# mbway/turbo

Hardware: AMD Instinct MI355X
Metric: acquisition evals/sec (M candidates, N training) + GP-fit ms (higher is better)
Workload: dtype f32

## Files before the change

turbo_amd/_lib.py:

```python
import ctypes
import importlib.util
import os
import sys

import numpy as np

_HERE = os.path.dirname(os.path.abspath(__file__))

os.environ.setdefault("GPU_MAX_HW_QUEUES", "8")
LIB_PATH = os.environ.get("TGP_LIBRARY") or os.path.join(_HERE, "csrc", "libturbogp.so")

OK, NOT_PD, BAD_ARG, HIP_ERROR, NOT_FITTED, NO_MEMORY, NO_DEVICE = 0, 1, 2, 3, 4, 5, 6
DEVICE_HOST = -1
F64, F32, F32X3, F32H2 = 0, 1, 2, 3
KERNELS = {"rbf": 0, "matern12": 1, "matern32": 2, "matern52": 3}
ACQ_NONE, ACQ_UCB, ACQ_PI, ACQ_EI, ACQ_SIGMA, ACQ_MES = 0, 1, 2, 3, 4, 5
BUF_K, BUF_L, BUF_LINV, BUF_ALPHA = 0, 1, 2, 3
BATCH_KB, BATCH_CL = 0, 1

SYMBOLS = (
    "tgp_create", "tgp_destroy", "tgp_last_error", "tgp_version", "tgp_fit", "tgp_fit_grad", "tgp_fit_optimise", "tgp_fit_lbfgsb", "tgp_set_private_stream",
    "tgp_set_overlap", "tgp_tuning", "tgp_mt19937_uniform_columns", "tgp_set_candidates_mt19937", "tgp_stream_status", "tgp_workers_acquire", "tgp_workers_release",
    "tgp_fit_append", "tgp_export_state", "tgp_import_state", "tgp_export_factor_dev", "tgp_import_factor_dev", "tgp_debug_read",
    "tgp_set_candidates", "tgp_set_candidates_dev", "tgp_gen_candidates", "tgp_gen_candidates_lhs", "tgp_lhs_design",
# ... 800 lines not shown

    def profile_enable(self, on=True):
        self._check(self.lib.tgp_profile_enable(self._h, 1 if on else 0))

    def profile_reset(self):
        self._check(self.lib.tgp_profile_reset(self._h))

    def profile_read(self):
        tl, kl = ctypes.c_int64(), ctypes.c_int64()
        tm, km, fm, sm = (ctypes.c_double() for _ in range(4))
        self._check(self.lib.tgp_profile_read(self._h, ctypes.byref(tl), ctypes.byref(tm),
                                              ctypes.byref(kl), ctypes.byref(km),
                                              ctypes.byref(fm), ctypes.byref(sm)))
        return dict(trmm_launches=tl.value, trmm_ms=tm.value, kstar_launches=kl.value,
                    kstar_ms=km.value, last_fit_ms=fm.value, last_sweep_ms=sm.value)

    def last_timings(self):
        v = np.zeros(12)
        self._check(self.lib.tgp_last_timings(self._h, _ptr(v), 12))
        return dict(fit_ms=v[0], sweep_ms=v[1], grad_kinv_ms=v[2], grad_pairwise_ms=v[3], grad_ard_ms=v[4],
                    trmm_flops=v[5], sweep_f64=int(v[6]), small_fit_phases_us=[float(x) for x in v[7:12]])

    def last_prune(self):
        v = np.zeros(17)
        self._check(self.lib.tgp_last_timings(self._h, _ptr(v), 17))
        return dict(state=int(v[12]), lb_set=int(v[13]), survivors=int(v[14]), screen=int(v[16]))

    def sweep_geometry(self):
        ch, npad = ctypes.c_int64(), ctypes.c_int64()
        self._check(self.lib.tgp_sweep_geometry(self._h, ctypes.byref(ch), ctypes.byref(npad)))
        return ch.value, npad.value
```

turbo_amd/csrc/sweep_kernels.hip:

```cpp
#include <hip/hip_runtime.h>
#include <math.h>
#include <stdlib.h>
#include <string.h>

#include "acq_math.hpp"
#include "mfma_gemm.hpp"
#include "pairwise.hpp"
#include "philox.hpp"
#include "prune_screen.hpp"
#include "tgp_internal.hpp"
#include "trmm_sweep.hpp"
#include "trmm_bf16x3.hpp"
#include "trmm_f16x2.hpp"

namespace tgp {

#define TGP_TRY(x)                         \
    do {                                   \
        hipError_t e_ = (x);               \
        if (e_ != hipSuccess) return e_;   \
    } while (0)

template <typename T>
__global__ __launch_bounds__(256) void prep_candidates_kernel(const double *__restrict__ Xc,
                                                              const double *__restrict__ ls,
                                                              T *__restrict__ Cs, long m_valid,
                                                              long rows, int D, int Dp) {
    const long total = rows * Dp;
    for (long i = (long)blockIdx.x * 256 + threadIdx.x; i < total; i += (long)gridDim.x * 256) {
        const long r = i / Dp;
        const int d = (int)(i - r * Dp);
        Cs[i] = (r < m_valid && d < D) ? (T)(Xc[r * D + d] / ls[d]) : (T)0;
// ... 595 lines not shown
    return hipSuccess;
}
template <typename T, int BK>
static hipError_t presweep_rows_t(Context &c, hipStream_t st, int rows_final, int budget128) {
    if (!c.pre.front) return hipSuccess;
    SweepPlan<T> p;
    TGP_TRY((make_plan<T, BK>(c, p)));
    int upto = rows_final / 128;
    if (upto > budget128) upto = budget128;
    upto &= ~1;
    if (upto > 2 * (p.nunits - 1)) upto = 2 * (p.nunits - 1);
    if (upto <= c.pre.rows128) return hipSuccess;
    const int tn = p.main.tile_n > 128 ? p.main.tile_n : 128;
    TGP_TRY(issue_trmm<T>(c, p, p.early, 0, 0, tn, c.pre.rows128, upto - c.pre.rows128, st));
    c.pre.rows128 = upto;
    return hipSuccess;
}

struct BoundArgs {
    const double *mupart, *abspart; long ldpart; int njs;
    long m;
    double err_scale;
    const double *err;
    double y_mean, y_std;
    double sig_lo, sig_hi;
    int acq; double sf, incumbent, param, margin;
    double *ub;
};

__global__ __launch_bounds__(256) void prune_bound_kernel(BoundArgs b) {
    const long c = (long)blockIdx.x * 256 + threadIdx.x;
    if (c >= b.m) return;
    double mun = 0.0, s = 0.0;
    for (int j = 0; j < b.njs; ++j) {
        mun += b.mupart[(long)j * b.ldpart + c];
        if (!b.err) s += b.abspart[(long)j * b.ldpart + c];
    }
    const double e = b.err ? b.err[c] : b.err_scale * s;
    const double mu = b.y_std * (b.sf > 0.0 ? mun + e : mun - e) + b.y_mean;
    const double a_lo = acq_value(b.acq, b.sf, b.incumbent, b.param, mu, b.sig_lo);
    const double a_hi = acq_value(b.acq, b.sf, b.incumbent, b.param, mu, b.sig_hi);
    double a = a_lo > a_hi ? a_lo : a_hi;
    double scale = fabs(a);
    if (b.acq == TGP_ACQ_UCB) scale += fabs(mu) + fabs(b.param) * b.sig_hi;
    a += b.margin * scale;
    b.ub[c] = (isnan(a_lo) || isnan(a_hi) || isnan(a)) ? INFINITY : a;
}

__global__ __launch_bounds__(256) void prune_pick_kernel(const double *__restrict__ ub, long m, long gs,
                                                         long long *__restrict__ pick) {
    __shared__ double sv[256];
    __shared__ long long si[256];
    const long g0 = (long)blockIdx.x * gs;
    const long g1 = g0 + gs < m ? g0 + gs : m;
    Best b;
    for (long c = g0 + threadIdx.x; c < g1; c += 256) {
        const double u = ub[c];
        if (u > b.v) { b.v = u; b.i = c; }
    }
    b = block_argmax<256>(b, sv, si);
    if (threadIdx.x == 0) pick[blockIdx.x] = b.i == IDX_NONE ? g0 : b.i;
// ... 51 lines not shown
        __syncthreads();
    }
    int run = part[threadIdx.x] - s;
    for (int b = b0; b < b1; ++b) { boff[b] = run; run += bcnt[b]; }
    if (threadIdx.x == 1023) total[0] = part[1023];
}

__global__ __launch_bounds__(256) void prune_scatter_kernel(SurvArgs s) {
    __shared__ int wsum[4];
    const long c = (long)blockIdx.x * 256 + threadIdx.x;
    const bool keep = prune_survives(s, c);
    const unsigned long long bal = __ballot(keep);
    const int lane = threadIdx.x & 63, w = threadIdx.x >> 6;
    if (lane == 0) wsum[w] = __popcll(bal);
    __syncthreads();
    int off = s.boff[blockIdx.x];
    for (int k = 0; k < w; ++k) off += wsum[k];
    if (keep) s.sidx[off + __popcll(bal & ((1ull << lane) - 1ull))] = s.src ? s.src[c] : c;
}

struct PruneWs {
    double *ub; long long *pick, *sidx, *misc; int *bcnt, *boff; void *cs;
    double *err, *ub1; long long *sidx1; float *nx;
};
static size_t al256(size_t b) { return (b + 255) & ~(size_t)255; }

template <typename T>
static hipError_t prune_workspace(Context &c, int64_t npick, int64_t rows_cap, bool screen, PruneWs &w) {
    const int64_t M = c.M, nb = (M + 255) / 256;
    const size_t o_pick = al256((size_t)M * 8), o_sidx = o_pick + al256((size_t)npick * 8), o_misc = o_sidx + al256((size_t)M * 8),
                 o_bcnt = o_misc + 256, o_boff = o_bcnt + al256((size_t)nb * 4), o_cs = o_boff + al256((size_t)nb * 4);
    const size_t o_err = o_cs + al256((size_t)rows_cap * c.Dp * sizeof(T));
    const size_t o_ub1 = o_err + (screen ? al256((size_t)c.ws_Mpad * 8) : 0), o_sidx1 = o_ub1 + (screen ? al256((size_t)rows_cap * 8) : 0),
                 o_nx = o_sidx1 + (screen ? al256((size_t)M * 8) : 0);
    const size_t need = o_nx + (screen ? al256((size_t)c.Np * 4) : 0);
    TGP_TRY(c.d_prune.reserve(need, [&] { return hipStreamSynchronize(c.stream); }));
    char *b = c.d_prune;
    w.ub = reinterpret_cast<double *>(b);
    w.pick = reinterpret_cast<long long *>(b + o_pick);
    w.sidx = reinterpret_cast<long long *>(b + o_sidx);
    w.misc = reinterpret_cast<long long *>(b + o_misc);
    w.bcnt = reinterpret_cast<int *>(b + o_bcnt);
    w.boff = reinterpret_cast<int *>(b + o_boff);
    w.cs = b + o_cs;
    w.err = reinterpret_cast<double *>(b + o_err);
    w.ub1 = reinterpret_cast<double *>(b + o_ub1);
    w.sidx1 = reinterpret_cast<long long *>(b + o_sidx1);
    w.nx = reinterpret_cast<float *>(b + o_nx);
    return hipSuccess;
}

template <typename T>
static TrmmVariant contract_variant(const SweepPlan<T> &p, int64_t rows, int ntm) {
    TrmmVariant v;
    v.kern = p.early.kern; v.lds = trmm_glds_lds_bytes(); v.tile_m = 128; v.tile_n = 128; v.threads = 256;
    if ((rows / 128) * ntm >= CONTRACT_MIN_WGS) return v;
    if ((rows / 64) * ntm >= CONTRACT_MIN_WGS) {
        v.kern = trmm_sumsq_glds_narrow_kernel<T, 64>; v.lds = trmm_narrow_lds_bytes<64>(); v.tile_n = 64;
    } else {
        v.kern = trmm_sumsq_glds_narrow_kernel<T, 32>; v.lds = trmm_narrow_lds_bytes<32>(); v.tile_n = 32;
    }
    return v;
}

template <typename T>
static hipError_t contract_rows(Context &c, const SweepPlan<T> &p, const T *cs, int64_t n, hipStream_t st, int &mark) {
    const int N = (int)c.N, Np = (int)c.Np, Dp = (int)c.Dp;
    constexpr int KAR = kstar_ar(sizeof(T));
    const T *Xs = reinterpret_cast<const T *>(sizeof(T) == 8 ? (const void *)c.d_Xs : (const void *)c.d_Xs32);
    const KstarFn<T> kst = kstar_fn<T>(c.kernel, false, false, true, false);
    for (int64_t off = 0; off < n; off += c.launch_rows) {
// ... 19 lines not shown
        TGP_TRY(hipGetLastError());
        m2 = prof_mark(c, st);
        prof_seg(c, mark, m2, 0, (double)m * (double)N * (double)N);
        mark = m2;
    }
    return hipSuccess;
}

template <typename T>
static hipError_t sweep_pruned(Context &c, const SweepPlan<T> &p, const SweepCall &call, bool front_usable, bool &done) {
    done = false;
    const int acq = call.acq;
    const double sf = call.sf, incumbent = call.incumbent, param = call.param;
    const Tuning &tu = tuning();
    const int64_t M = c.M, Mpad = c.ws_Mpad;
    const int N = (int)c.N, Dp = (int)c.Dp;
    hipStream_t st = c.stream;
    const int64_t top = tu.prune_top < 1 ? 1 : tu.prune_top;
    const int64_t gs = (M + top - 1) / top, npick = (M + gs - 1) / gs;
    const double frac = tuning_prune_frac_now();
    const int64_t keep = frac < 0.0 ? -1 : (frac >= 1.0 ? M : (int64_t)(frac * (double)M));
    const int64_t rows_cap = (((npick > keep ? npick : keep) + 127) / 128) * 128;
    const bool screen = sizeof(T) == 4 && c.kernel == TGP_RBF && c.D <= SCR_MAXD && tuning_prune_screen_now() != 0;
    PruneWs w;
    TGP_TRY(prune_workspace<T>(c, npick, rows_cap, screen, w));
    TGP_TRY(lds_opt_in(c, p.early.kern, p.early.lds));
    const T *Cs = reinterpret_cast<const T *>(c.d_Cs.get());
    const T *Xs = reinterpret_cast<const T *>(sizeof(T) == 8 ? (const void *)c.d_Xs : (const void *)c.d_Xs32);
    T *cs = reinterpret_cast<T *>(w.cs);
    constexpr int KAR = kstar_ar(sizeof(T));
    c.prune_screen = -1;

    if (!front_usable) TGP_TRY(issue_prep<T>(c, st));
    int mark = prof_mark(c, st);

    BoundArgs b{};
    b.mupart = c.d_mupart; b.abspart = c.d_part; b.ldpart = Mpad;
    b.err_scale = 4.0 * (double)(N + 8) * 0x1p-53;
    b.y_mean = c.y_mean; b.y_std = c.y_std;
    b.sig_lo = sqrt((0.99 * c.noise) * (c.y_std * c.y_std));
    b.sig_hi = sqrt((c.constant + c.noise) * (c.y_std * c.y_std));
    b.acq = acq; b.sf = sf; b.incumbent = incumbent; b.param = param; b.margin = tu.prune_margin;

    auto tight_bound = [&](const T *rowsrc, int64_t rows, int64_t m, double *ub) -> hipError_t {
        const int64_t xb = rows / (16 * KAR);
        int njs_b = 1;
        while (njs_b < p.njs && xb * njs_b < BOUND_MIN_WGS) njs_b *= 2;
        if (njs_b > p.njs) njs_b = p.njs;
        hipLaunchKernelGGL(kstar_fn<T>(c.kernel, false, false, false, true), dim3((unsigned)xb, (unsigned)njs_b),
                           dim3(256), 0, st, rowsrc, Xs, c.d_alpha, reinterpret_cast<T *>(c.d_part.get()), c.d_mupart, (int)rows, N,
                           (int)c.Np, Dp, c.constant, (long)Mpad, 0L, 1.f);
        TGP_TRY(hipGetLastError());
        const int m2 = prof_mark(c, st);
        prof_seg(c, mark, m2, 1);
        mark = m2;
        b.njs = njs_b; b.m = m; b.err = nullptr; b.ub = ub;
        hipLaunchKernelGGL(prune_bound_kernel, dim3((unsigned)((m + 255) / 256)), dim3(256), 0, st, b);
        return hipGetLastError();
    };

    if (screen) {
        if constexpr (sizeof(T) == 4) {
            const ScreenTerms et = screen_error_terms(c.constant, (int)c.D, N);
            double *scal = reinterpret_cast<double *>(w.misc + 8);
            hipLaunchKernelGGL(screen_stats_kernel, dim3(1), dim3(1024), 0, st, Xs, c.d_alpha, N, (int)c.Np, Dp, et.P, et.Q, w.nx, scal);
            TGP_TRY(hipGetLastError());
            const int m1 = prof_mark(c, st);
            const int64_t xb = Mpad / SCR_T;
            const int njt = (N + SCR_T - 1) / SCR_T;
            int njs_s = 1;
            while (njs_s < p.njs && njs_s < njt && xb * njs_s < SCREEN_MIN_WGS) njs_s *= 2;
            if (njs_s > p.njs) njs_s = p.njs;
            ScreenArgs g{};
            g.Cs = Cs; g.Xs = Xs; g.alpha = c.d_alpha; g.nx = w.nx; g.scal = scal;
            g.mupart = c.d_mupart; g.err = w.err; g.ldpart = Mpad;
            g.N = N; g.Np = (int)c.Np; g.Dp = Dp; g.constant = c.constant;
            hipLaunchKernelGGL(prune_screen_kernel, dim3((unsigned)xb, (unsigned)njs_s), dim3(256), 0, st, g);
            TGP_TRY(hipGetLastError());
            const int m2 = prof_mark(c, st);
            prof_seg(c, m1, m2, 2);
            mark = m2;
            b.njs = njs_s; b.m = M; b.err = w.err; b.ub = w.ub;
            hipLaunchKernelGGL(prune_bound_kernel, dim3((unsigned)((M + 255) / 256)), dim3(256), 0, st, b);
            TGP_TRY(hipGetLastError());
        }
    } else {
        TGP_TRY(tight_bound(Cs, Mpad, M, w.ub));
    }
    hipLaunchKernelGGL(prune_pick_kernel, dim3((unsigned)npick), dim3(256), 0, st, w.ub, (long)M, (long)gs, w.pick);
    TGP_TRY(hipGetLastError());

    auto gather = [&](const long long *idx, int64_t n) -> hipError_t {
        const long total = (long)(((n + 127) / 128) * 128) * Dp;
        const long blocks = (total + 255) / 256 < 8192 ? (total + 255) / 256 : 8192;
        hipLaunchKernelGGL(prune_gather_kernel<T>, dim3((unsigned)blocks), dim3(256), 0, st, Cs, Dp, idx, (long)n,
                           (long)(((n + 127) / 128) * 128), cs);
        return hipGetLastError();
    };
    auto finalize = [&](const long long *idx, int64_t n, int64_t blk0) -> hipError_t {
        FinArgs f{};
        f.part = c.d_part; f.ldpart = Mpad;
        f.nunits = p.nunits; f.n128 = p.n128;
        f.base_pairs = p.nunits;
        f.mupart = c.d_mupart; f.njs = 1;
// ... 198 lines not shown
```

turbo_amd/csrc/tgp_api.hip:

```cpp
#include <hip/hip_runtime.h>
#include <math.h>
#include <stdlib.h>
#include <string.h>

#include <algorithm>
#include <atomic>
#include <chrono>
#include <condition_variable>
#include <functional>
#include <mutex>
#include <new>
#include <string>
#include <system_error>
#include <thread>
#include <vector>

#include "host_backend.hpp"
#include "host_lbfgsb.hpp"
#include "host_slice.hpp"
#include "tgp_internal.hpp"

using namespace tgp;

struct tgp_handle_s {
// ... 1293 lines not shown
}

static int winner_mark(Context &c, const SweepCall &s) {
    if (!s.winner || s.acq == TGP_ACQ_NONE) return TGP_OK;
    API_HIP(c.ev_winner.create(hipEventDisableTiming), "hipEventCreate");
    API_HIP(hipEventRecord(c.ev_winner, c.stream), "hipEventRecord");
    c.winner_recorded = true;
    return TGP_OK;
}

static int run_sweep(Context &c, const SweepCall &call, CallClock &clk) {
    SweepCall s = call;
    if (s.acq == TGP_ACQ_MES) s.mes = MesArgs{c.d_mes, c.mes_S, c.noise * (c.y_std * c.y_std)};
    const SweepPath path = sweep_path(c, c.M);
    int rc = path == SweepPath::General ? ensure_workspace(c) : ensure_small_workspace(c);
    if (rc != TGP_OK) return rc;
    const bool front = path == SweepPath::General && s.may_use_front && c.pre.gen == c.fit_gen && c.pre.cand == c.d_cand &&
                       c.pre.M == c.M && c.pre.Mpad == c.ws_Mpad && c.pre.launch_rows == c.launch_rows && c.pre.chunk == c.chunk;
    c.pre.front = false;
    c.last_sweep_f64 = path != SweepPath::General || c.dtype == TGP_F64;
    c.prune_state = -1;
    c.prune_lbset = c.prune_surv = 0;
    c.prune_screen = -1;
    if ((rc = call_begin(c, clk)) != TGP_OK) return rc;
    hipError_t le;
    if (path == SweepPath::OneLaunch) {
        le = launch_mid_sweep(c, s);
    } else if (path == SweepPath::OneWorkgroup) {
        le = launch_small_sweep(c, s);
        if (le == hipSuccess) le = launch_argmax_final(c, s);
    } else {
        le = launch_sweep(c, s, front);
    }
    if (le != hipSuccess) return hip_fail(c, le, "launch_sweep");
    return winner_mark(c, s);
}

struct SweepRecord { double bv = 0.0; long long bi[2] = {0, 0}; };
static int sweep_queue_return(Context &c, bool zc, int acq, SweepRecord &r, CallClock *clk, double *mu, double *sigma, double *acq_out) {
    if (!zc) {
        if (acq != TGP_ACQ_NONE) API_HIP(hipMemcpyAsync(&r.bv, c.d_best, sizeof(double), hipMemcpyDeviceToHost, c.stream), "D2H best");
        API_HIP(hipMemcpyAsync(r.bi, c.d_besti, 2 * sizeof(long long), hipMemcpyDeviceToHost, c.stream), "D2H besti");
        API_HIP(hipMemsetAsync(c.d_besti, 0, 4 * sizeof(long long), c.stream), "memset counters");
    }
    if (clk) API_MEM(call_stop(c, *clk));
    const size_t bytes = (size_t)c.M * sizeof(double);
// ... 1283 lines not shown
        if (last_sweep_ms) *last_sweep_ms = h->host->last_sweep_ms;
        return TGP_OK;
    }
    Context &c = h->c;
    prof_collect(c);
    if (trmm_launches) *trmm_launches = c.trmm_launches;
    if (trmm_ms) *trmm_ms = c.trmm_ms;
    if (kstar_launches) *kstar_launches = c.kstar_launches;
    if (kstar_ms) *kstar_ms = c.kstar_ms;
    if (last_fit_ms) *last_fit_ms = c.last_fit_ms;
    if (last_sweep_ms) *last_sweep_ms = c.last_sweep_ms;
    return TGP_OK;
} TGP_CATCH

int tgp_last_timings(tgp_handle h, double *out, int64_t n) try {
    if (!h) return TGP_BAD_ARG;
    if (h->host) {
        if (!out || n < 1) { h->host->err = "tgp_last_timings: need out and n >= 1"; return TGP_BAD_ARG; }
        for (int64_t i = 0; i < n; ++i) out[i] = i == 0 ? h->host->last_fit_ms : (i == 1 ? h->host->last_sweep_ms : (i == 6 ? 1.0 : (i == 12 || i == 16 ? -1.0 : 0.0)));
        return TGP_OK;
    }
    Context &c = h->c;
    if (!out || n < 1) return fail(c, TGP_BAD_ARG, "tgp_last_timings: need out and n >= 1");
    double v[18] = {c.last_fit_ms, c.last_sweep_ms, c.last_grad_ms[0], c.last_grad_ms[1], c.last_grad_ms[2], c.trmm_flops,
                    (double)c.last_sweep_f64, 0.0, 0.0, 0.0, 0.0, 0.0, (double)c.prune_state, (double)c.prune_lbset,
                    (double)c.prune_surv, c.last_cov_ms, (double)c.prune_screen, c.screen_ms};
    if (c.h_bell && c.h_bell[1]) {
        const unsigned long long t0 = c.h_bell[1];
        const int src[5] = {3, 4, 5, 6, 2};
        for (int k = 0; k < 5; ++k) v[7 + k] = c.h_bell[src[k]] >= t0 ? (double)(c.h_bell[src[k]] - t0) * 1e-2 : 0.0;
    }
    for (int64_t i = 0; i < n; ++i) out[i] = i < 18 ? v[i] : 0.0;
    return TGP_OK;
} TGP_CATCH

int tgp_sweep_geometry(tgp_handle h, int64_t *chunk, int64_t *n_padded) try {
    if (!h) return TGP_BAD_ARG;
    if (h->host) { if (chunk) *chunk = 16; if (n_padded) *n_padded = h->host->N; return TGP_OK; }
    if (chunk) *chunk = h->c.chunk;
    if (n_padded) *n_padded = h->c.Np;
    return TGP_OK;
} TGP_CATCH

}
```

turbo_amd/csrc/tgp_internal.hpp:

```cpp
#pragma once
#include <hip/hip_runtime.h>
#include <stdint.h>

#include <string>
#include <vector>

#include "../../include/turbogp.h"
#include "dev_mem.hpp"
#include "doorbell.hpp"
#include "lds_opt_in.hpp"
#include "mes_math.hpp"
#include "tuning.hpp"

namespace tgp {


constexpr int NB = 64;
constexpr int NPAD = 256;
constexpr int SW_BM = 128;
constexpr int SW_BN = 128;
constexpr int KS_JS = 8;
constexpr int FIN_BLOCK = 256;
constexpr int CONTRACT_MIN_WGS = 512;
constexpr int SCREEN_MIN_WGS = 1024;
// ... 111 lines not shown
    int64_t fit_gen_src = -1;

    bool small = false;
    int64_t linv_extent = 0;
    Pin<double> h_pin_in{hipHostMallocMapped | hipHostMallocCoherent};
    Pin<double> h_pin_out{hipHostMallocMapped | hipHostMallocCoherent};
    Pin<double> h_pin_cand{hipHostMallocMapped};
    Pin<uint32_t> h_mt_words{hipHostMallocDefault, false};
    Ev ev_mt[2];
    Pin<unsigned long long> h_bell{hipHostMallocMapped | hipHostMallocCoherent};
    unsigned long long bell_seq = 0;
    Dev<unsigned> d_ticket;
    Dev<double> d_sfg;

    const double *d_cand = nullptr;
    Dev<double> d_cand_owned;
    int64_t M = 0;

    int64_t chunk = 0;
    int64_t launch_rows = 0;
    int prune_state = -1;
    int64_t prune_lbset = 0, prune_surv = 0;
    int64_t prune_screen = -1;
    double screen_ms = 0.0;
    Dev<double> d_bval;
    Dev<long long> d_bidx;
    double *d_winner = nullptr;
    int64_t winner_offset = 0;
    Ev ev_winner;
    bool winner_recorded = false;
    Dev<double> d_best;
    Dev<long long> d_besti;

    bool profiling = false;
    std::vector<Ev> ev_pool;
    size_t ev_used = 0;
    std::vector<ProfSeg> segs;
    int64_t trmm_launches = 0, kstar_launches = 0;
    double trmm_ms = 0.0, kstar_ms = 0.0;
    double trmm_flops = 0.0;
    double last_fit_ms = 0.0, last_sweep_ms = 0.0;
    int last_sweep_f64 = -1;
};

hipStream_t private_fit_begin(int device, bool may_borrow);
void private_fit_end(int device, bool held);
// ... 170 lines not shown
```

turbo_amd/csrc/tuning.hpp:

```cpp
#pragma once
#include <stdio.h>
#include <stdlib.h>
#include <string.h>

#include <string>

namespace tgp {

#define TGP_TUNING_TABLE(X)                                                                                                      \
                                                                          \
    X(INT, chunk, "TGP_CHUNK", 0, "candidates per slab group (multiple of 1024; 0 = about 256 MiB of slab) [per call]")          \
    X(DBL, slab_gb, "TGP_SLAB_GB", 1.0, "GiB of cross-kernel slab per launch pair (groups of TGP_CHUNK inside it)")              \
    X(STR, tile, "TGP_TILE", "", "contraction tile: 128 | 256x128 | 256x256 (default: by launch size)")                         \
    X(INT, nbuf, "TGP_NBUF", 0, "LDS k-tile buffers of the 256x128 contraction: 2 | 3 (default: 3 for f64, 2 for f32)")          \
    X(STR, trmm, "TGP_TRMM", "", "reg = the register-staged contraction template instead of the direct-to-LDS kernels (A/B)")    \
    X(INT, bk, "TGP_BK", 0, "k-tile of the contraction (f32: 16 | 32 | 64, f64: 8 | 16 | 32); other than 128 bytes = template")  \
    X(INT, mfma16, "TGP_MFMA16", 0, "1 = v_mfma_f32_16x16x4 fragments in the 128-tile f32 contraction")                         \
    X(INT, ks_js, "TGP_KS_JS", 0, "splits of the training points over the cross-kernel grid (0 = up to 8)")                       \
    X(INT, sweep_zc, "TGP_SWEEP_ZC", 1, "0 = the sweep's result record by D2H copies + memset instead of mapped host memory")    \
    X(INT, mean_in_trmm, "TGP_MEAN", 1, "1 = posterior mean K*.alpha accumulated inside the contraction's full-k row tiles (f64 / f32); 0 = in the cross-kernel (round 4)") \
    X(INT, overlap, "TGP_OVERLAP", 2, "sweep started inside tgp_fit for the resident batch: 0 = never, 1 = scaling + first cross-kernel, 2 = + contraction row tiles whose rows of Linv are final") \
    X(INT, pre_tiles, "TGP_PRE_TILES", -1, "128-row tiles of the first launch pair contracted inside the fit in mode 2 (-1 = a quarter of the rows)") \
    X(INT, pre_cus, "TGP_PRE_CUS", -1, "CUs of the third stream, which carries the sweep's front inside a fit (-1 = three quarters of the device, 0 = unmasked)") \
    X(INT, pre_cu0, "TGP_PRE_CU0", 0, "first CU of that mask")                                                                 \
    X(INT, pre_lds_kb, "TGP_PRE_LDS_KB", 81, "KiB of LDS requested per workgroup of the early contraction (64 = two per CU, 81 = one)") \
    X(INT, sweep_prune, "TGP_SWEEP_PRUNE", 1, "1 = an arg-max-only EI / PI / UCB sweep (f32 / f64, N > 256) contracts only the candidates whose acquisition bound can still win (sweep_pruned); 0 = every candidate [per call]") \
    X(INT, prune_top, "TGP_PRUNE_TOP", 256, "candidates of the pruned sweep's lb set (the best bound of each of this many groups): its best exact value is the bar") \
    X(DBL, prune_frac, "TGP_PRUNE_FRAC", 0.25, "the pruned sweep runs the full schedule when more than this share of the batch survives (< 0: always) [per call]") \
    X(DBL, prune_min_work, "TGP_PRUNE_MIN_WORK", 1e11, "the pruned sweep runs only when M * N^2 (the full contraction's multiply-adds) reaches this: below, its fixed cost is more than it saves [per call]") \
    X(DBL, prune_tau, "TGP_PRUNE_TAU", 2e4, "the pruned sweep needs s^2 / (c + s^2) >= this * the contraction's unit roundoff (no skipped candidate can clamp)") \
    X(INT, prune_screen, "TGP_PRUNE_SCREEN", 1, "1 = the pruned sweep of an f32 RBF handle screens every candidate on the matrix cores first (prune_screen.hpp) and runs its tight bound pass only on the screen's survivors; 0 = the tight bound pass over all candidates [per call]") \
    X(INT, prune_direct, "TGP_PRUNE_DIRECT", 1024, "screen survivors up to this many are contracted as they are; more (up to TGP_PRUNE_FRAC of the batch) go through the tight bound pass first [per call]") \
    X(DBL, prune_margin, "TGP_PRUNE_MARGIN", 1e-6, "relative slack of the pruned sweep's bounds against the bar (rounding of the acquisition formulas)") \
    X(INT, mid, "TGP_MID", 1, "0 = 128 < N <= 256 down the general sweep instead of the one-launch kernel")                      \
    X(INT, mid_maxm, "TGP_MID_MAXM", 0, "largest batch that takes the one-launch sweep for 256 < N <= 512 (0 = never) [per call]") \
    X(INT, small, "TGP_SMALL", 1, "0 = N <= 128 down the blocked path instead of the one-workgroup kernels")                     \
                                                                         \
    X(INT, ob, "TGP_OB", 0, "outer block of the Cholesky (multiple of 256; 0 = by size: all of Np <= 1024, else 256 / 512 / 1024)") \
    X(INT, panel, "TGP_PANEL", 5, "diagonal-block factorisation: 5 = variant D (LDS block, MFMA), 3 / 38 = C, 4 / 8 = B, 0 = round 1") \
    X(INT, panel_la, "TGP_PANEL_LA", 1, "0 = pivot factored in the panel launch instead of beside the previous update")          \
    X(INT, panel_fuse, "TGP_PANEL_FUSE", 1, "0 = two launches per panel instead of fused_panel_kernel")                          \
    X(INT, panel_fuse_tiles, "TGP_PANEL_FUSE_TILES", 384, "fused panel launches for outer blocks whose first update has at most this many tiles") \
    X(STR, inner, "TGP_INNER", "", "gemm64 = the in-block rank-64 update on the generic template")                               \
    X(STR, gemm64, "TGP_GEMM64", "", "reg = the f64 64x64 NT products on the register-staged template (A/B, bit-identical)")     \
    X(INT, trail64, "TGP_TRAIL64", 8192, "trailing updates of up to this many rows on 64x64 tiles (beyond: 128-tile kernel)")    \
    X(INT, merge64, "TGP_MERGE64", 2048, "inverse merges with a leading block up to this on 64x64 tiles")                        \
    X(INT, kinv64, "TGP_KINV64", 4096, "K^-1 = U U^T of the LML gradient on 64x64 tiles up to this Np")                          \
    X(INT, bginv, "TGP_BGINV", 1, "0 = the inverse level by level after the factorisation instead of behind the panel chain")   \
    X(INT, level64_fused, "TGP_LEVEL64_FUSED", 1, "0 = the 64 -> 128 level of the inverse as three launches (two products + transpose) instead of one") \
    X(INT, bginv_max, "TGP_BGINV_MAX", 9216, "largest Np whose inverse runs behind the chain")                                   \
    X(INT, bg_lease, "TGP_BG_LEASE", 1, "0 = a fit on a private stream never borrows the background stream (its inverse always in line)") \
    X(INT, bg_cus, "TGP_BG_CUS", -1, "CUs of the background stream (-1 = three quarters of the device, 0 = unmasked)")           \
    X(INT, bg_probe, "TGP_BG_PROBE", 1, "0 = skip the probe that the stream pair really overlaps")                               \
    X(INT, linv_zero, "TGP_LINV_ZERO", 0, "1 = every fit zero-fills Linv (default: only when it may hold stale rows)")           \
// ... 51 lines not shown
        out += buf;                                                     \
    }
        TGP_TUNING_TABLE(TGP_TD)
#undef TGP_TD
#undef TGP_TD_INT
#undef TGP_TD_DBL
#undef TGP_TD_STR
        return out;
    }
};

inline const Tuning &tuning() {
    static const Tuning t;
    return t;
}

inline int runtime_hw_queues_env() { const char *v = getenv("GPU_MAX_HW_QUEUES"); return v ? atoi(v) : 0; }

inline int tuning_chunk_now() { const char *v = getenv("TGP_CHUNK"); return v ? atoi(v) : 0; }
inline int tuning_mid_maxm_now() { const char *v = getenv("TGP_MID_MAXM"); return v ? atoi(v) : 0; }
inline int tuning_sweep_prune_now() { const char *v = getenv("TGP_SWEEP_PRUNE"); return v ? atoi(v) : 1; }
inline double tuning_prune_frac_now() { const char *v = getenv("TGP_PRUNE_FRAC"); return v ? atof(v) : 0.25; }
inline int tuning_prune_screen_now() { const char *v = getenv("TGP_PRUNE_SCREEN"); return v ? atoi(v) : 1; }
inline int tuning_prune_direct_now() { const char *v = getenv("TGP_PRUNE_DIRECT"); return v ? atoi(v) : 1024; }
inline double tuning_prune_min_work_now() { const char *v = getenv("TGP_PRUNE_MIN_WORK"); return v ? atof(v) : 1e11; }

}
```

Baseline: 71.49 million.

## Screen pruned-sweep candidates with split-fp16 MFMA and a kernel-weighted error bound

Adds a new screening kernel for the pruned sweep. It splits candidate and training coordinates into two fp16 planes and computes the cross products with v_mfma_f32_32x32x16_f16. Training rows are pre-sorted by the sign of alpha so that positive and negative contributions accumulate separately. The new error bound combines the closed-form bound with a k-weighted bound, which should let more candidates be pruned. It is the default for D >= 15 and adds a prep launch and extra workspace, with the risk that the fp16 error bounds are loose or wrong.

```diff
diff --git a/turbo_amd/_lib.py b/turbo_amd/_lib.py
--- a/turbo_amd/_lib.py
+++ b/turbo_amd/_lib.py
@@ -846,9 +846,9 @@
                     trmm_flops=v[5], sweep_f64=int(v[6]), small_fit_phases_us=[float(x) for x in v[7:12]])
 
     def last_prune(self):
-        v = np.zeros(17)
-        self._check(self.lib.tgp_last_timings(self._h, _ptr(v), 17))
-        return dict(state=int(v[12]), lb_set=int(v[13]), survivors=int(v[14]), screen=int(v[16]))
+        v = np.zeros(19)
+        self._check(self.lib.tgp_last_timings(self._h, _ptr(v), 19))
+        return dict(state=int(v[12]), lb_set=int(v[13]), survivors=int(v[14]), screen=int(v[16]), screen_arith=int(v[18]))
 
     def sweep_geometry(self):
         ch, npad = ctypes.c_int64(), ctypes.c_int64()
diff --git a/turbo_amd/csrc/prune_screen_h2.hpp b/turbo_amd/csrc/prune_screen_h2.hpp
--- /dev/null
+++ b/turbo_amd/csrc/prune_screen_h2.hpp
@@ -0,0 +1,342 @@
+#pragma once
+#include <hip/hip_runtime.h>
+#include <math.h>
+
+#include "prune_screen.hpp"
+#include "trmm_f16x2.hpp"
+
+namespace tgp {
+
+constexpr int SCRH_MIN_D = 15;
+constexpr int SCRH_ROW = 144;
+constexpr int SCRH_MAXEXP = 40;
+
+struct ScreenH2Terms { double dcoef, P, Qc, Qw; };
+inline ScreenH2Terms screen_h2_error_terms(double constant, int D, int N) {
+    const double u = 0x1p-24, ce = 1.001 * constant, L = fabs(log2(constant));
+    ScreenH2Terms t;
+    t.dcoef = 2.01 * D + 25.0 + 0.26 * sqrt((double)D);
+    t.P = ce * u * 0.5 * t.dcoef;
+    t.Qc = screen_error_terms(constant, D, N).Q + ce * (0.7 * L * u + 0x1p-41);
+    t.Qw = t.Qc + ce * u * (2.4 + 1.4 * L);
+    return t;
+}
+
+__host__ __device__ inline double screen_h2_weight(double dcoef, double R) {
+    const double delta = dcoef * 0x1p-24 * R + 0x1p-40;
+    return delta <= 1.0 ? 1.001 * expm1(0.5001 * delta) : INFINITY;
+}
+__host__ __device__ inline double screen_h2_error(double closed, double wcoef, double W, double wadd) {
+    return fmin(closed, wcoef * W + wadd);
+}
+
+__host__ __device__ inline float screen_h2_scale(float m) {
+    int e;
+    frexpf(m, &e);
+    int ex = 14 - e;
+    ex = ex > SCRH_MAXEXP ? SCRH_MAXEXP : (ex < -SCRH_MAXEXP ? -SCRH_MAXEXP : ex);
+    return ldexpf(1.f, ex);
+}
+
+struct ScreenH2Scal {
+    double ea, eb, wadd;
+    float nxmax, sx;
+    int npos, nneg, ok, pad;
+};
+
+struct ScreenH2PrepArgs {
+    const float *Xs;
+    const double *alpha;
+    int N, Dp, nch;
+    long ncap;
+    double P, Qc, Qw;
+    unsigned char *Xh;
+    float *nxp, *absa;
+    ScreenH2Scal *scal;
+};
+
+__global__ __launch_bounds__(256) void screen_h2_prep_kernel(ScreenH2PrepArgs a) {
+    __shared__ double sa[256];
+    __shared__ float smx[256], smn[256];
+    __shared__ int spos[256], sbef[256], sbad[256];
+    __shared__ int wcnt[4];
+    const int tid = threadIdx.x, base = blockIdx.x * 256;
+    const int N = a.N, Dp = a.Dp;
+    double a1 = 0.0;
+    float mxx = 0.f, mxn = 0.f;
+    int npos = 0, before = 0, bad = 0;
+    for (int i = tid; i < N; i += 256) {
+        const float *row = a.Xs + (long)i * Dp;
+        double s = 0.0;
+        float m = 0.f;
+        for (int d = 0; d < Dp; d += 4) {
+            const f4_t x = *reinterpret_cast<const f4_t *>(row + d);
+#pragma unroll
+            for (int e = 0; e < 4; ++e) { s = fma((double)x[e], (double)x[e], s); m = fmaxf(m, fabsf(x[e])); }
+        }
+        if (!(s < (double)INFINITY)) bad = 1;
+        mxn = fmaxf(mxn, (float)s);
+        mxx = fmaxf(mxx, m);
+        const double al = a.alpha[i];
+        a1 += fabs(al);
+        const int p = al >= 0.0;
+        npos += p;
+        if (i < base) before += p;
+    }
+    sa[tid] = a1; smx[tid] = mxx; smn[tid] = mxn; spos[tid] = npos; sbef[tid] = before; sbad[tid] = bad;
+    __syncthreads();
+    for (int o = 128; o > 0; o >>= 1) {
+        if (tid < o) {
+            sa[tid] += sa[tid + o];
+            smx[tid] = fmaxf(smx[tid], smx[tid + o]);
+            smn[tid] = fmaxf(smn[tid], smn[tid + o]);
+            spos[tid] += spos[tid + o];
+            sbef[tid] += sbef[tid + o];
+            sbad[tid] |= sbad[tid + o];
+        }
+        __syncthreads();
+    }
+    npos = spos[0];
+    before = sbef[0];
+    const int nneg = N - npos, np128 = (npos + 127) & ~127, nn128 = (nneg + 127) & ~127;
+    const float xm2 = 2.f * smx[0];
+    const float sx = xm2 > 0.f ? screen_h2_scale(xm2) : 1.f;
+    const int ok = !sbad[0] && xm2 < 0x1p54f;
+    if (blockIdx.x == 0 && tid == 0) {
+        const double an = 1.001 * sa[0];
+        ScreenH2Scal s;
+        s.ea = an * (a.P * (double)smn[0] + a.Qc);
+        s.eb = an * a.P;
+        s.wadd = an * a.Qw;
+        s.nxmax = smn[0]; s.sx = sx;
+        s.npos = npos; s.nneg = nneg; s.ok = ok; s.pad = 0;
+        *a.scal = s;
+    }
+
+    const int i = base + tid;
+    const bool live = i < N;
+    const double al = live ? a.alpha[i] : -1.0;
+    const bool pos = live && al >= 0.0;
+    const unsigned long long bal = __ballot(pos);
+    const int lane = tid & 63, w = tid >> 6;
+    if (lane == 0) wcnt[w] = __popcll(bal);
+    __syncthreads();
+    int pre = __popcll(bal & ((1ull << lane) - 1ull));
+    for (int k = 0; k < w; ++k) pre += wcnt[k];
+    auto write_row = [&](long dest, const float *row, float absal) {
+        double s = 0.0;
+        for (int ch = 0; ch < a.nch; ++ch) {
+            unsigned h[2][16];
+#pragma unroll
+            for (int q = 0; q < 8; ++q) {
+                const int d = ch * SCR_DC + 4 * q;
+                f4_t x = {0.f, 0.f, 0.f, 0.f};
+                if (row && d < Dp) x = *reinterpret_cast<const f4_t *>(row + d);
+#pragma unroll
+                for (int e = 0; e < 4; ++e) s = fma((double)x[e], (double)x[e], s);
+                split2_f16x2(-2.f * x[0], -2.f * x[1], sx, h[0][2 * q], h[1][2 * q]);
+                split2_f16x2(-2.f * x[2], -2.f * x[3], sx, h[0][2 * q + 1], h[1][2 * q + 1]);
+            }
+            unsigned char *o = a.Xh + ((long)ch * a.ncap + dest) * 128;
+#pragma unroll
+            for (int pl = 0; pl < 2; ++pl)
+#pragma unroll
+                for (int q = 0; q < 4; ++q)
+                    *reinterpret_cast<u4_t *>(o + 64 * pl + 16 * q) = (u4_t){h[pl][4 * q], h[pl][4 * q + 1], h[pl][4 * q + 2], h[pl][4 * q + 3]};
+        }
+        a.nxp[dest] = (float)s;
+        a.absa[dest] = absal;
+    };
+    if (live) write_row(pos ? before + pre : np128 + (i - before - pre), a.Xs + (long)i * Dp, (float)fabs(al));
+    if (blockIdx.x == 0 && tid < 128) {
+        if (npos + tid < np128) write_row(npos + tid, nullptr, 0.f);
+        if (nneg + tid < nn128) write_row(np128 + nneg + tid, nullptr, 0.f);
+    }
+}
+
+struct ScreenH2Args {
+    const float *Cs;
+    const unsigned char *Xh;
+    const float *nxp, *absa;
+    const ScreenH2Scal *scal;
+    double *mupart, *wpart;
+    double *err, *wcoef;
+    long ldpart, ncap;
+    int Dp;
+    double constant, dcoef;
+};
+
+__global__ __launch_bounds__(256, 2) void prune_screen_h2_kernel(ScreenH2Args g) {
+    __shared__ __attribute__((aligned(16))) unsigned char Ct[SCR_T * SCRH_ROW];
+    __shared__ __attribute__((aligned(16))) unsigned char Xt[SCR_T * SCRH_ROW];
+    __shared__ __attribute__((aligned(16))) f4_t rowc[SCR_T];
+    __shared__ float srow[SCR_T];
+    __shared__ double mpos[SCR_T];
+    const int tid = threadIdx.x, lane = tid & 63, w = tid >> 6;
+    const int li = lane & 31, lh = lane >> 5;
+    const long c0 = (long)blockIdx.x * SCR_T;
+    const int Dp = g.Dp;
+    const ScreenH2Scal sc = *g.scal;
+    const int ntp = (sc.npos + SCR_T - 1) / SCR_T;
+    const int njt = ntp + (sc.nneg + SCR_T - 1) / SCR_T;
+    const int per = (njt + (int)gridDim.y - 1) / (int)gridDim.y;
+    const int jt0 = blockIdx.y * per;
+    const int jt1 = jt0 + per < njt ? jt0 + per : njt;
+    const int nch = (Dp + SCR_DC - 1) / SCR_DC;
+    const int nsteps = (jt1 > jt0 ? jt1 - jt0 : 0) * nch;
+    const bool one_pass = nch == 1;
+    constexpr float KAPPA = -0.72134752044448170368f;
+
+    if (tid < SCR_T) {
+        const float *row = g.Cs + (c0 + tid) * Dp;
+        double s = 0.0;
+        float m = 0.f;
+        for (int d = 0; d < Dp; d += 4) {
+            const f4_t x = *reinterpret_cast<const f4_t *>(row + d);
+#pragma unroll
+            for (int e = 0; e < 4; ++e) { s = fma((double)x[e], (double)x[e], s); m = fmaxf(m, fabsf(x[e])); }
+        }
+        const double R = s + (double)sc.nxmax;
+        const bool ok = sc.ok && R < 0x1p46;
+        const float sr = ok ? (m > 0.f ? screen_h2_scale(m) : 1.f) : 0.f;
+        const float S = sr * sc.sx;
+        srow[tid] = sr;
+        rowc[tid] = (f4_t){S, KAPPA / S, (float)((double)log2f((float)g.constant) + (double)KAPPA * s), -(float)((double)S * s)};
+        if (blockIdx.y == 0) {
+            g.err[c0 + tid] = ok ? sc.ea + sc.eb * s : (double)INFINITY;
+            g.wcoef[c0 + tid] = ok ? screen_h2_weight(g.dcoef, R) : (double)INFINITY;
+        }
+    }
+    __syncthreads();
+    ScrStage sp;
+    u4_t xq[4];
+    auto store_c = [&]() {
+#pragma unroll
+        for (int p = 0; p < 4; ++p) {
+            const int idx = tid + 256 * p;
+            const int r = idx >> 3, dv = (idx & 7) * 4;
+            const float sr = srow[r];
+            unsigned a0, a1, b0, b1;
+            split2_f16x2(sp.v[p][0], sp.v[p][1], sr, a0, b0);
+            split2_f16x2(sp.v[p][2], sp.v[p][3], sr, a1, b1);
+            *reinterpret_cast<uint2 *>(Ct + r * SCRH_ROW + 2 * dv) = make_uint2(a0, a1);
+            *reinterpret_cast<uint2 *>(Ct + r * SCRH_ROW + 64 + 2 * dv) = make_uint2(b0, b1);
+        }
+    };
+    auto load_x = [&](int jt, int ch) {
+        const unsigned char *src = g.Xh + ((long)ch * g.ncap + (long)jt * SCR_T) * 128;
+#pragma unroll
+        for (int p = 0; p < 4; ++p) xq[p] = *reinterpret_cast<const u4_t *>(src + (tid + 256 * p) * 16);
+    };
+    auto store_x = [&]() {
+#pragma unroll
+        for (int p = 0; p < 4; ++p) {
+            const int idx = tid + 256 * p;
+            *reinterpret_cast<u4_t *>(Xt + (idx >> 3) * SCRH_ROW + (idx & 7) * 16) = xq[p];
+        }
+    };
+    if (nsteps > 0) {
+        sp.load(g.Cs, c0, Dp, 0);
+        load_x(jt0, 0);
+        store_c();
+        store_x();
+    }
+    __syncthreads();
+    double sum[16];
+#pragma unroll
+    for (int r = 0; r < 16; ++r) sum[r] = 0.0;
+    auto mma = [](u4_t a, u4_t b, f16_t c) {
+        return __builtin_amdgcn_mfma_f32_32x32x16_f16(__builtin_bit_cast(f16x8_t, a), __builtin_bit_cast(f16x8_t, b), c, 0, 0, 0);
+    };
+    f16_t hi[4], mid[4];
+    for (int st = 0; st < nsteps; ++st) {
+        const int jt = jt0 + st / nch, ch = st - (st / nch) * nch;
+        const int j0 = jt * SCR_T;
+        const bool more = st + 1 < nsteps;
+        if (more) {
+            const int jn = jt0 + (st + 1) / nch, cn = (st + 1) - ((st + 1) / nch) * nch;
+            load_x(jn, cn);
+        }
+        float nxv[4], al[4];
+        if (ch == nch - 1) {
+#pragma unroll
+            for (int b = 0; b < 4; ++b) {
+                nxv[b] = g.nxp[j0 + 32 * b + li];
+                al[b] = g.absa[j0 + 32 * b + li];
+            }
+        }
+        if (ch == 0) {
+            if (jt == ntp && jt > jt0) {
+#pragma unroll
+                for (int r = 0; r < 16; ++r) {
+                    double s = sum[r];
+#pragma unroll
+                    for (int o = 16; o > 0; o >>= 1) s += __shfl_xor(s, o, 64);
+                    if (li == 0) mpos[32 * w + Mfma<float>::c_row(lane, r)] = s;
+                    sum[r] = 0.0;
+                }
+            }
+#pragma unroll
+            for (int b = 0; b < 4; ++b)
+#pragma unroll
+                for (int r = 0; r < 16; ++r) { hi[b][r] = 0.f; mid[b][r] = 0.f; }
+        }
+        int dn = Dp - ch * SCR_DC;
+        if (dn > SCR_DC) dn = SCR_DC;
+        const int nkb = (dn + 15) >> 4;
+#pragma unroll 1
+        for (int kb = 0; kb < nkb; ++kb) {
+            const int off = 32 * kb + 16 * lh;
+            const unsigned char *ap = Ct + (32 * w + li) * SCRH_ROW + off;
+            const u4_t a1 = *reinterpret_cast<const u4_t *>(ap), a2 = *reinterpret_cast<const u4_t *>(ap + 64);
+#pragma unroll
+            for (int b = 0; b < 4; ++b) {
+                const unsigned char *bp = Xt + (32 * b + li) * SCRH_ROW + off;
+                const u4_t b1 = *reinterpret_cast<const u4_t *>(bp), b2 = *reinterpret_cast<const u4_t *>(bp + 64);
+                hi[b] = mma(a1, b1, hi[b]);
+                mid[b] = mma(a1, b2, mid[b]);
+                mid[b] = mma(a2, b1, mid[b]);
+            }
+        }
+        if (ch == nch - 1) {
+#pragma unroll
+            for (int r = 0; r < 16; ++r) {
+                const f4_t rc = rowc[32 * w + Mfma<float>::c_row(lane, r)];
+                float p = 0.f;
+#pragma unroll
+                for (int b = 0; b < 4; ++b) {
+                    const float t = fmaf(mid[b][r], 0x1p-11f, hi[b][r]);
+                    const float s = fmaxf(fmaf(nxv[b], rc[0], t), rc[3]);
+                    const float kv = __builtin_amdgcn_exp2f(fmaf(s, rc[1], rc[2]));
+                    p = b == 0 ? kv * al[0] : fmaf(kv, al[b], p);
+                }
+                sum[r] += (double)p;
+            }
+        }
+        if (more) {
+            __syncthreads();
+            if (!one_pass) {
+                sp.load(g.Cs, c0, Dp, ((st + 1) - ((st + 1) / nch) * nch) * SCR_DC);
+                store_c();
+            }
+            store_x();
+            __syncthreads();
+        }
+    }
+    const bool has_pos = nsteps > 0 && jt0 < ntp, has_neg = nsteps > 0 && jt1 > ntp;
+#pragma unroll
+    for (int r = 0; r < 16; ++r) {
+        double s = sum[r];
+#pragma unroll
+        for (int o = 16; o > 0; o >>= 1) s += __shfl_xor(s, o, 64);
+        if (li == 0) {
+            const int row = 32 * w + Mfma<float>::c_row(lane, r);
+            const double mp = has_neg ? (has_pos ? mpos[row] : 0.0) : s, mn = has_neg ? s : 0.0;
+            const long o = (long)blockIdx.y * g.ldpart + c0 + row;
+            g.mupart[o] = mp - mn;
+            g.wpart[o] = mp + mn;
+        }
+    }
+}
+
+}
diff --git a/turbo_amd/csrc/sweep_kernels.hip b/turbo_amd/csrc/sweep_kernels.hip
--- a/turbo_amd/csrc/sweep_kernels.hip
+++ b/turbo_amd/csrc/sweep_kernels.hip
@@ -8,6 +8,7 @@
 #include "pairwise.hpp"
 #include "philox.hpp"
 #include "prune_screen.hpp"
+#include "prune_screen_h2.hpp"
 #include "tgp_internal.hpp"
 #include "trmm_sweep.hpp"
 #include "trmm_bf16x3.hpp"
@@ -649,6 +650,8 @@
     long m;
     double err_scale;
     const double *err;
+    const double *wcoef;
+    const double *wadd;
     double y_mean, y_std;
     double sig_lo, sig_hi;
     int acq; double sf, incumbent, param, margin;
@@ -661,9 +664,10 @@
     double mun = 0.0, s = 0.0;
     for (int j = 0; j < b.njs; ++j) {
         mun += b.mupart[(long)j * b.ldpart + c];
-        if (!b.err) s += b.abspart[(long)j * b.ldpart + c];
-    }
-    const double e = b.err ? b.err[c] : b.err_scale * s;
+        if (!b.err || b.wcoef) s += b.abspart[(long)j * b.ldpart + c];
+    }
+    double e = b.err ? b.err[c] : b.err_scale * s;
+    if (b.wcoef) e = screen_h2_error(e, b.wcoef[c], s, b.wadd[0]);
     const double mu = b.y_std * (b.sf > 0.0 ? mun + e : mun - e) + b.y_mean;
     const double a_lo = acq_value(b.acq, b.sf, b.incumbent, b.param, mu, b.sig_lo);
     const double a_hi = acq_value(b.acq, b.sf, b.incumbent, b.param, mu, b.sig_hi);
@@ -761,18 +765,22 @@
 struct PruneWs {
     double *ub; long long *pick, *sidx, *misc; int *bcnt, *boff; void *cs;
     double *err, *ub1; long long *sidx1; float *nx;
+    double *wcoef; unsigned char *xh; float *nxp, *absa; long ncap;
 };
 static size_t al256(size_t b) { return (b + 255) & ~(size_t)255; }
 
 template <typename T>
-static hipError_t prune_workspace(Context &c, int64_t npick, int64_t rows_cap, bool screen, PruneWs &w) {
+static hipError_t prune_workspace(Context &c, int64_t npick, int64_t rows_cap, bool screen, bool h2, PruneWs &w) {
     const int64_t M = c.M, nb = (M + 255) / 256;
     const size_t o_pick = al256((size_t)M * 8), o_sidx = o_pick + al256((size_t)npick * 8), o_misc = o_sidx + al256((size_t)M * 8),
                  o_bcnt = o_misc + 256, o_boff = o_bcnt + al256((size_t)nb * 4), o_cs = o_boff + al256((size_t)nb * 4);
     const size_t o_err = o_cs + al256((size_t)rows_cap * c.Dp * sizeof(T));
     const size_t o_ub1 = o_err + (screen ? al256((size_t)c.ws_Mpad * 8) : 0), o_sidx1 = o_ub1 + (screen ? al256((size_t)rows_cap * 8) : 0),
                  o_nx = o_sidx1 + (screen ? al256((size_t)M * 8) : 0);
-    const size_t need = o_nx + (screen ? al256((size_t)c.Np * 4) : 0);
+    const long ncap = (long)((c.N + SCR_T - 1) / SCR_T + 1) * SCR_T, nch = (long)((c.Dp + SCR_DC - 1) / SCR_DC);
+    const size_t o_wc = o_nx + (screen ? al256((size_t)c.Np * 4) : 0), o_xh = o_wc + (h2 ? al256((size_t)c.ws_Mpad * 8) : 0),
+                 o_nxp = o_xh + (h2 ? al256((size_t)nch * ncap * 128) : 0), o_absa = o_nxp + (h2 ? al256((size_t)ncap * 4) : 0);
+    const size_t need = o_absa + (h2 ? al256((size_t)ncap * 4) : 0);
     TGP_TRY(c.d_prune.reserve(need, [&] { return hipStreamSynchronize(c.stream); }));
     char *b = c.d_prune;
     w.ub = reinterpret_cast<double *>(b);
@@ -786,6 +794,11 @@
     w.ub1 = reinterpret_cast<double *>(b + o_ub1);
     w.sidx1 = reinterpret_cast<long long *>(b + o_sidx1);
     w.nx = reinterpret_cast<float *>(b + o_nx);
+    w.wcoef = reinterpret_cast<double *>(b + o_wc);
+    w.xh = reinterpret_cast<unsigned char *>(b + o_xh);
+    w.nxp = reinterpret_cast<float *>(b + o_nxp);
+    w.absa = reinterpret_cast<float *>(b + o_absa);
+    w.ncap = ncap;
     return hipSuccess;
 }
 
@@ -851,14 +864,16 @@
     const int64_t keep = frac < 0.0 ? -1 : (frac >= 1.0 ? M : (int64_t)(frac * (double)M));
     const int64_t rows_cap = (((npick > keep ? npick : keep) + 127) / 128) * 128;
     const bool screen = sizeof(T) == 4 && c.kernel == TGP_RBF && c.D <= SCR_MAXD && tuning_prune_screen_now() != 0;
+    const bool h2 = screen && tuning_screen_arith_now() == 2 && c.D >= SCRH_MIN_D;
     PruneWs w;
-    TGP_TRY(prune_workspace<T>(c, npick, rows_cap, screen, w));
+    TGP_TRY(prune_workspace<T>(c, npick, rows_cap, screen, h2, w));
     TGP_TRY(lds_opt_in(c, p.early.kern, p.early.lds));
     const T *Cs = reinterpret_cast<const T *>(c.d_Cs.get());
     const T *Xs = reinterpret_cast<const T *>(sizeof(T) == 8 ? (const void *)c.d_Xs : (const void *)c.d_Xs32);
     T *cs = reinterpret_cast<T *>(w.cs);
     constexpr int KAR = kstar_ar(sizeof(T));
     c.prune_screen = -1;
+    c.prune_arith = 0;
 
     if (!front_usable) TGP_TRY(issue_prep<T>(c, st));
     int mark = prof_mark(c, st);
@@ -883,32 +898,58 @@
         const int m2 = prof_mark(c, st);
         prof_seg(c, mark, m2, 1);
         mark = m2;
-        b.njs = njs_b; b.m = m; b.err = nullptr; b.ub = ub;
+        b.njs = njs_b; b.m = m; b.err = nullptr; b.wcoef = nullptr; b.ub = ub;
         hipLaunchKernelGGL(prune_bound_kernel, dim3((unsigned)((m + 255) / 256)), dim3(256), 0, st, b);
         return hipGetLastError();
     };
 
     if (screen) {
         if constexpr (sizeof(T) == 4) {
-            const ScreenTerms et = screen_error_terms(c.constant, (int)c.D, N);
-            double *scal = reinterpret_cast<double *>(w.misc + 8);
-            hipLaunchKernelGGL(screen_stats_kernel, dim3(1), dim3(1024), 0, st, Xs, c.d_alpha, N, (int)c.Np, Dp, et.P, et.Q, w.nx, scal);
-            TGP_TRY(hipGetLastError());
-            const int m1 = prof_mark(c, st);
             const int64_t xb = Mpad / SCR_T;
             const int njt = (N + SCR_T - 1) / SCR_T;
             int njs_s = 1;
             while (njs_s < p.njs && njs_s < njt && xb * njs_s < SCREEN_MIN_WGS) njs_s *= 2;
             if (njs_s > p.njs) njs_s = p.njs;
-            ScreenArgs g{};
-            g.Cs = Cs; g.Xs = Xs; g.alpha = c.d_alpha; g.nx = w.nx; g.scal = scal;
-            g.mupart = c.d_mupart; g.err = w.err; g.ldpart = Mpad;
-            g.N = N; g.Np = (int)c.Np; g.Dp = Dp; g.constant = c.constant;
-            hipLaunchKernelGGL(prune_screen_kernel, dim3((unsigned)xb, (unsigned)njs_s), dim3(256), 0, st, g);
-            TGP_TRY(hipGetLastError());
-            const int m2 = prof_mark(c, st);
-            prof_seg(c, m1, m2, 2);
-            mark = m2;
+            if (h2) {
+                const ScreenH2Terms et = screen_h2_error_terms(c.constant, (int)c.D, N);
+                ScreenH2Scal *scal = reinterpret_cast<ScreenH2Scal *>(w.misc + 8);
+                static_assert(sizeof(ScreenH2Scal) <= 256 - 64, "the scalars live behind misc's first eight words");
+                ScreenH2PrepArgs a{};
+                a.Xs = Xs; a.alpha = c.d_alpha; a.N = N; a.Dp = Dp; a.nch = (Dp + SCR_DC - 1) / SCR_DC; a.ncap = w.ncap;
+                a.P = et.P; a.Qc = et.Qc; a.Qw = et.Qw;
+                a.Xh = w.xh; a.nxp = w.nxp; a.absa = w.absa; a.scal = scal;
+                hipLaunchKernelGGL(screen_h2_prep_kernel, dim3((unsigned)((N + 255) / 256)), dim3(256), 0, st, a);
+                TGP_TRY(hipGetLastError());
+                const int m1 = prof_mark(c, st);
+                ScreenH2Args g{};
+                g.Cs = Cs; g.Xh = w.xh; g.nxp = w.nxp; g.absa = w.absa; g.scal = scal;
+                g.mupart = c.d_mupart; g.wpart = c.d_part; g.err = w.err; g.wcoef = w.wcoef; g.ldpart = Mpad; g.ncap = w.ncap;
+                g.Dp = Dp; g.constant = c.constant; g.dcoef = et.dcoef;
+                hipLaunchKernelGGL(prune_screen_h2_kernel, dim3((unsigned)xb, (unsigned)njs_s), dim3(256), 0, st, g);
+                TGP_TRY(hipGetLastError());
+                const int m2 = prof_mark(c, st);
+                prof_seg(c, m1, m2, 2);
+                mark = m2;
+                c.prune_arith = 2;
+                b.wcoef = w.wcoef; b.wadd = &scal->wadd;
+            } else {
+                const ScreenTerms et = screen_error_terms(c.constant, (int)c.D, N);
+                double *scal = reinterpret_cast<double *>(w.misc + 8);
+                hipLaunchKernelGGL(screen_stats_kernel, dim3(1), dim3(1024), 0, st, Xs, c.d_alpha, N, (int)c.Np, Dp, et.P, et.Q, w.nx, scal);
+                TGP_TRY(hipGetLastError());
+                const int m1 = prof_mark(c, st);
+                ScreenArgs g{};
+                g.Cs = Cs; g.Xs = Xs; g.alpha = c.d_alpha; g.nx = w.nx; g.scal = scal;
+                g.mupart = c.d_mupart; g.err = w.err; g.ldpart = Mpad;
+                g.N = N; g.Np = (int)c.Np; g.Dp = Dp; g.constant = c.constant;
+                hipLaunchKernelGGL(prune_screen_kernel, dim3((unsigned)xb, (unsigned)njs_s), dim3(256), 0, st, g);
+                TGP_TRY(hipGetLastError());
+                const int m2 = prof_mark(c, st);
+                prof_seg(c, m1, m2, 2);
+                mark = m2;
+                c.prune_arith = 1;
+                b.wcoef = nullptr;
+            }
             b.njs = njs_s; b.m = M; b.err = w.err; b.ub = w.ub;
             hipLaunchKernelGGL(prune_bound_kernel, dim3((unsigned)((M + 255) / 256)), dim3(256), 0, st, b);
             TGP_TRY(hipGetLastError());
diff --git a/turbo_amd/csrc/tgp_api.hip b/turbo_amd/csrc/tgp_api.hip
--- a/turbo_amd/csrc/tgp_api.hip
+++ b/turbo_amd/csrc/tgp_api.hip
@@ -1339,6 +1339,7 @@
     c.prune_state = -1;
     c.prune_lbset = c.prune_surv = 0;
     c.prune_screen = -1;
+    c.prune_arith = 0;
     if ((rc = call_begin(c, clk)) != TGP_OK) return rc;
     hipError_t le;
     if (path == SweepPath::OneLaunch) {
@@ -2668,15 +2669,15 @@
     }
     Context &c = h->c;
     if (!out || n < 1) return fail(c, TGP_BAD_ARG, "tgp_last_timings: need out and n >= 1");
-    double v[18] = {c.last_fit_ms, c.last_sweep_ms, c.last_grad_ms[0], c.last_grad_ms[1], c.last_grad_ms[2], c.trmm_flops,
+    double v[19] = {c.last_fit_ms, c.last_sweep_ms, c.last_grad_ms[0], c.last_grad_ms[1], c.last_grad_ms[2], c.trmm_flops,
                     (double)c.last_sweep_f64, 0.0, 0.0, 0.0, 0.0, 0.0, (double)c.prune_state, (double)c.prune_lbset,
-                    (double)c.prune_surv, c.last_cov_ms, (double)c.prune_screen, c.screen_ms};
+                    (double)c.prune_surv, c.last_cov_ms, (double)c.prune_screen, c.screen_ms, (double)c.prune_arith};
     if (c.h_bell && c.h_bell[1]) {
         const unsigned long long t0 = c.h_bell[1];
         const int src[5] = {3, 4, 5, 6, 2};
         for (int k = 0; k < 5; ++k) v[7 + k] = c.h_bell[src[k]] >= t0 ? (double)(c.h_bell[src[k]] - t0) * 1e-2 : 0.0;
     }
-    for (int64_t i = 0; i < n; ++i) out[i] = i < 18 ? v[i] : 0.0;
+    for (int64_t i = 0; i < n; ++i) out[i] = i < 19 ? v[i] : 0.0;
     return TGP_OK;
 } TGP_CATCH
 
diff --git a/turbo_amd/csrc/tgp_internal.hpp b/turbo_amd/csrc/tgp_internal.hpp
--- a/turbo_amd/csrc/tgp_internal.hpp
+++ b/turbo_amd/csrc/tgp_internal.hpp
@@ -157,6 +157,7 @@
     int prune_state = -1;
     int64_t prune_lbset = 0, prune_surv = 0;
     int64_t prune_screen = -1;
+    int prune_arith = 0;
     double screen_ms = 0.0;
     Dev<double> d_bval;
     Dev<long long> d_bidx;
diff --git a/turbo_amd/csrc/tuning.hpp b/turbo_amd/csrc/tuning.hpp
--- a/turbo_amd/csrc/tuning.hpp
+++ b/turbo_amd/csrc/tuning.hpp
@@ -30,6 +30,7 @@
     X(DBL, prune_min_work, "TGP_PRUNE_MIN_WORK", 1e11, "the pruned sweep runs only when M * N^2 (the full contraction's multiply-adds) reaches this: below, its fixed cost is more than it saves [per call]") \
     X(DBL, prune_tau, "TGP_PRUNE_TAU", 2e4, "the pruned sweep needs s^2 / (c + s^2) >= this * the contraction's unit roundoff (no skipped candidate can clamp)") \
     X(INT, prune_screen, "TGP_PRUNE_SCREEN", 1, "1 = the pruned sweep of an f32 RBF handle screens every candidate on the matrix cores first (prune_screen.hpp) and runs its tight bound pass only on the screen's survivors; 0 = the tight bound pass over all candidates [per call]") \
+    X(STR, screen_arith, "TGP_SCREEN_ARITH", "h2", "arithmetic of that screen: h2 = two fp16 planes per operand on v_mfma_f32_32x32x16_f16 and a k-weighted error (prune_screen_h2.hpp; D >= 15, else f32), f32 = prune_screen.hpp's kernel and closed form; the A/B switch [per call]") \
     X(INT, prune_direct, "TGP_PRUNE_DIRECT", 1024, "screen survivors up to this many are contracted as they are; more (up to TGP_PRUNE_FRAC of the batch) go through the tight bound pass first [per call]") \
     X(DBL, prune_margin, "TGP_PRUNE_MARGIN", 1e-6, "relative slack of the pruned sweep's bounds against the bar (rounding of the acquisition formulas)") \
     X(INT, mid, "TGP_MID", 1, "0 = 128 < N <= 256 down the general sweep instead of the one-launch kernel")                      \
@@ -127,6 +128,7 @@
 inline int tuning_sweep_prune_now() { const char *v = getenv("TGP_SWEEP_PRUNE"); return v ? atoi(v) : 1; }
 inline double tuning_prune_frac_now() { const char *v = getenv("TGP_PRUNE_FRAC"); return v ? atof(v) : 0.25; }
 inline int tuning_prune_screen_now() { const char *v = getenv("TGP_PRUNE_SCREEN"); return v ? atoi(v) : 1; }
+inline int tuning_screen_arith_now() { const char *v = getenv("TGP_SCREEN_ARITH"); return v && !strcmp(v, "f32") ? 1 : 2; }
 inline int tuning_prune_direct_now() { const char *v = getenv("TGP_PRUNE_DIRECT"); return v ? atoi(v) : 1024; }
 inline double tuning_prune_min_work_now() { const char *v = getenv("TGP_PRUNE_MIN_WORK"); return v ? atof(v) : 1e11; }
 
```

Result: faster. 82.32 million, median of 6 (+15.1%).
